# mjmyt/drone_path_planning_python

Measured on AMD Instinct MI355X. Metric: minimum-snap trajectories/sec (N drones × M segments, order 7) at 1/2/4/8 MI355X, higher is better.
Workload: dtype f64

## Files before the change

### drone_path_planning_python_amd/csrc/msnap_solve.hip

```cpp
#include "msnap_consts.h"
#include <cstdlib>

#include "msnap_internal.h"
#include "msnap_dispatch.h"
#include "msnap_sweep.h"
#include "msnap_rolled.h"

namespace msnap {


template <int K, bool GS>
__global__ void __launch_bounds__(kWave)
solve_kernel(const double *__restrict__ wp, const double *__restrict__ tt, int shared_times,
             int N, int M, double *__restrict__ coef, double *__restrict__ dur,
             int32_t *__restrict__ status, double *__restrict__ gscratch, int ntiles) {
  constexpr int NU = K - 1, NC = 2 * K;

  extern __shared__ __attribute__((aligned(16))) double lds[];

  const int lane = threadIdx.x;
  const int knots = M - 1;
  const int wpitch = (M + 1) * 4;
  const int tpitch = M + 1;

// ... 276 lines not shown
    for (int n = MCOL; n < NU; ++n) OtG[sidx(n, MCOL)] = quad_bcast<MCOL>(col[n]);
    twin_gather<NU, NS, MCOL + 1>(col, OtG);
  }
}

template <int K, int M>
__global__ void __launch_bounds__(kWave, (kTwinWaves<K, M>))
solve_kernel_twin(const double *__restrict__ wp, const double *__restrict__ tt, int shared_times,
                  int N, double *__restrict__ coef, double *__restrict__ dur,
                  int32_t *__restrict__ status, int ntiles) {
  using SW = Sweep<K>;
  using C = HermiteConsts<K>;
  constexpr int NU = SW::NU, NC = SW::NC, NS = SW::NS, KK = SW::KK, PM = SW::PM;
  static_assert(NU <= kAxes && NU >= 3, "one column of the knot blocks per axis lane (order 7: the fourth lane idles through the column work)");
  static_assert(M >= 4, "both sides own at least one knot");
  constexpr int kSlotWords = NU * kWave;
  constexpr int nL = (M - 2) / 2, nR = (M - 2) - nL;
  constexpr int H = nR;
  constexpr bool kAsym = nL != nR;
  constexpr int HA = H > 0 ? H : 1;

  extern __shared__ __attribute__((aligned(16))) double lds[];

  const int lane0 = threadIdx.x;
  constexpr int wpitch = (M + 1) * 4;
  constexpr int tpitch = M + 1;
  double *sWraw = lds;
  double *sTraw = sWraw + kTwinDrones * wpitch;
  double2 *sTr = reinterpret_cast<double2 *>(lds);
  double *sG = lds + (NC == 10 ? kTwinTrWords : 0);
  constexpr int ZL = kTwinZInLds<K, M>;
  double *sZ = sG + H * kSlotWords;
  double dsg[NU];
#pragma unroll
  for (int r = 0; r < NU; ++r) dsg[r] = (r & 1) ? 1.0 : -1.0;

  auto tile_valid = [&](int tl) {
    const int left = N - tl * kTwinDrones;
    return left < kTwinDrones ? left : kTwinDrones;
  };
  static_assert(nL >= 1, "the prefetch sits in front of segments 1 and 0 of the backward sweep, which both sides own");
  constexpr int kStoresPerSeg = (NC == 8 ? 4 : NC / 2);
  TwinStage<M> pre;
  if ((int)blockIdx.x < ntiles)
    twin_stage_load<M>(wp, tt, shared_times, blockIdx.x, tile_valid(blockIdx.x), lane0, pre);
  wait_vmcnt<0>();

  for (int tile = blockIdx.x; tile < ntiles; tile += gridDim.x) {
    int lane = lane0;
    asm volatile("" : "+v"(lane));
    const int a = lane & 3;
    const int side = (lane >> 2) & 1;
    const int blk = lane >> 2;
    const int dl = lane >> 3;
    double ca[NU];
#pragma unroll
    for (int n = 0; n < NU; ++n)
      ca[n] = a == 0 ? C::HSE[n + 1][1] : a == 1 ? C::HSE[n + 1][2] : a == 2 ? C::HSE[n + 1][3] : C::HSE[n + 1][NU];
    const int d_raw = tile * kTwinDrones + dl;
    const bool live = d_raw < N;
    const int d = live ? d_raw : N - 1;
    const int nvalid = tile_valid(tile);
    const int next = tile + gridDim.x;

    asm volatile("s_setprio 0" ::: "memory");
    wave_lds_fence();
    twin_stage_wait<M, 2 * kStoresPerSeg>(pre);
    twin_stage_store<M>(shared_times, nvalid, sWraw, sTraw, lane, pre);
    wave_lds_fence();
    store_durations(sTraw, shared_times, tpitch, M, nvalid, lane, dur + (size_t)tile * kTwinDrones * M);

    const int dloc = live ? dl : (N - 1 - tile * kTwinDrones);
    const double *lw = sWraw + dloc * wpitch + a;
    const double *lt = sTraw + (shared_times ? 0 : dloc * tpitch);
    auto Wown = [&](int i) -> double { return lw[(side ? M - i : i) * 4]; };
    auto Town = [&](int i) -> double {
      const int j = side ? M - 1 - i : i;
      return lt[j + 1] - lt[j];
    };

    double wreg[HA + 2], xreg[HA + 1], zreg[HA][NU];
    const double t0 = lt[0];
    bool nonfinite = !finite64(t0);
    bool badtime = t0 < 0.0;
#pragma unroll
    for (int i = 0; i <= H + 1; ++i) {
      wreg[i] = Wown(i);
      nonfinite |= !finite64(wreg[i]);
    }
#pragma unroll
    for (int i = 0; i <= H; ++i) {
      double T = Town(i);
      nonfinite |= !finite64(T);
      badtime |= !(T > 0.0);
      if (i == 0) {
        T = side ? T : T - t0;
        badtime |= !(T > 0.0);
      }
      xreg[i] = rcp64(T);
    }
    int in_flags = (nonfinite ? 4 : 0) | (badtime ? 2 : 0);
    asm volatile("" : "+v"(in_flags));
    wave_lds_fence();

    double xpp[PM], rz[NU], OtG[NS];
    {
      double xp[PM + 1];
      SW::powers(xreg[0], xp);
      const double dw0 = wreg[1] - wreg[0];
#pragma unroll
      for (int p = 1; p <= PM; ++p) xpp[p - 1] = xp[p];
#pragma unroll
      for (int n = 1; n <= NU; ++n) rz[n - 1] = C::HEE[n][0] * (xp[KK - n] * dw0);
#pragma unroll
      for (int e = 0; e < NS; ++e) OtG[e] = 0.0;
    }
#pragma unroll
    for (int it = 1; it <= H; ++it) {
      double xpp0[PM], rz0[NU], OtG0[NS];
      if (kAsym && it == H) {
#pragma unroll
        for (int p = 0; p < PM; ++p) xpp0[p] = xpp[p];
#pragma unroll
        for (int r = 0; r < NU; ++r) rz0[r] = rz[r];
#pragma unroll
        for (int e = 0; e < NS; ++e) OtG0[e] = OtG[e];
      }
      double xp[PM + 1];
      SW::powers(xreg[it], xp);
      const double dw = wreg[it + 1] - wreg[it];
      double S[NS], y[NU];
#pragma unroll
      for (int n = 1; n <= NU; ++n)
#pragma unroll
        for (int m = 1; m <= n; ++m)
          S[sidx(n - 1, m - 1)] =
              __builtin_fma(C::HSS[n][m], xp[KK - n - m],
                            __builtin_fma(C::HEE[n][m], xpp[KK - n - m - 1], -OtG[sidx(n - 1, m - 1)]));
#pragma unroll
      for (int n = 1; n <= NU; ++n) {
        const double tdw = xp[KK - n] * dw;
        y[n - 1] = __builtin_fma(-C::HSE[n][0], tdw, -rz[n - 1]);
        rz[n - 1] = C::HEE[n][0] * tdw;
      }
      double dinv[NU];
      in_flags |= (SW::ldl_factor(S, dinv) && (!kAsym || it <= nL || side)) ? 1 : 0;
      asm volatile("" : "+v"(in_flags));
      const double pa = a == 0 ? xp[NU] : a == 1 ? xp[NU - 1] : a == 2 ? xp[NU - 2] : xp[NU - 3];
      double g[NU];
#pragma unroll
      for (int n = 0; n < NU; ++n) g[n] = ca[n] * (n == NU - 1 ? pa : pa * xp[NU - 1 - n]);
      SW::ldl_solve(S, dinv, g);
      SW::ldl_solve(S, dinv, y);
      {
        double *gs = sG + (it - 1) * kSlotWords + lane;
#pragma unroll
        for (int r = 0; r < NU; ++r) gs[r * kWave] = g[r];
      }
      if (it <= ZL) {
#pragma unroll
        for (int r = 0; r < NU; ++r) sZ[((it - 1) * NU + r) * kWave + lane] = y[r];
      } else {
#pragma unroll
        for (int r = 0; r < NU; ++r) zreg[it - 1][r] = y[r];
      }
#pragma unroll
      for (int q = 0; q < NU - 1; ++q) {
        g[q] *= xp[NU - 1 - q];
        y[q] *= xp[NU - 1 - q];
      }
      double col[NU];
#pragma unroll
      for (int n = 0; n < NU; ++n) {
        double sg = C::HSE[1][n + 1] * g[0], sz = C::HSE[1][n + 1] * y[0];
#pragma unroll
        for (int q = 1; q < NU; ++q) {
          sg = __builtin_fma(C::HSE[q + 1][n + 1], g[q], sg);
          sz = __builtin_fma(C::HSE[q + 1][n + 1], y[q], sz);
        }
        col[n] = sg * xp[NU - n];
        rz[n] = __builtin_fma(sz, xp[NU - n], rz[n]);
      }
      twin_gather<NU, NS>(col, OtG);
#pragma unroll
      for (int p = 1; p <= PM; ++p) xpp[p - 1] = xp[p];
      if (kAsym && it == H) {
#pragma unroll
        for (int p = 0; p < PM; ++p) xpp[p] = side ? xpp[p] : xpp0[p];
#pragma unroll
        for (int r = 0; r < NU; ++r) rz[r] = side ? rz[r] : rz0[r];
#pragma unroll
        for (int e = 0; e < NS; ++e) OtG[e] = side ? OtG[e] : OtG0[e];
      }
    }

    double Sm[NS], um[NU];
#pragma unroll
    for (int r = 0; r < NU; ++r) {
      const double q = rz[r];
      um[r] = -q - dsg[r] * __shfl_xor(q, 4);
#pragma unroll
      for (int c = 0; c <= r; ++c) {
        const double p = __builtin_fma(C::HEE[r + 1][c + 1], xpp[KK - r - c - 3], -OtG[sidx(r, c)]);
        Sm[sidx(r, c)] = p + (dsg[r] * dsg[c]) * __shfl_xor(p, 4);
      }
    }
    {
      double dinv[NU];
      in_flags |= SW::ldl_factor(Sm, dinv) ? 1 : 0;
      SW::ldl_solve(Sm, dinv, um);
    }

    const int gsh = lane & ~7;
    const bool f_nonfinite = ((__ballot((in_flags & 4) != 0) >> gsh) & 0xFFull) != 0;
    const bool f_time = ((__ballot((in_flags & 2) != 0) >> gsh) & 0xFFull) != 0;
    const bool f_sing = ((__ballot((in_flags & 1) != 0) >> gsh) & 0xFFull) != 0;
    const int st = f_nonfinite ? MSNAP_ST_NONFINITE : f_time ? MSNAP_ST_TIMES : f_sing ? MSNAP_ST_SINGULAR : MSNAP_ST_OK;
    if (live && (lane & 7) == 0) status[d] = st;
    const bool bad = st != 0;

    const double qnan = __builtin_nan("");
    const double zero_or_nan = bad ? qnan : 0.0;
    TwinStorePlan plan;
    if constexpr (NC == 10) twin_store_plan(lane, plan);
    double *blkp = coef + ((size_t)d * M + (side ? M - 1 - H : H)) * (4 * NC) + (NC == 10 ? a * 2 : 0);
    const int blkstep = side ? 4 * NC : -(4 * NC);
#pragma unroll
    for (int i = 0; i < H + 2; ++i) wreg[i] = bad ? qnan : wreg[i];
    double un[NU];
#pragma unroll
    for (int r = 0; r < NU; ++r) un[r] = bad ? qnan : um[r];
#pragma unroll
    for (int it = H; it >= 0; --it) {
      if (it != 1) __builtin_amdgcn_sched_barrier(0);
      if (it == 1) {
        __builtin_amdgcn_sched_barrier(0);
        const int nx = next < ntiles ? next : ntiles - 1;
        twin_stage_load<M>(wp, tt, shared_times, nx, tile_valid(nx), lane, pre);
      }
      const bool own = !kAsym || it <= nL || side != 0;
      double u[NU];
      if (it >= 1) {
        const double2 *gsl = reinterpret_cast<const double2 *>(sG + (it - 1) * kSlotWords + blk * kAxes);
#pragma unroll
        for (int r = 0; r < NU; ++r) {
          const double2 g01 = gsl[r * (kWave / 2)], g23 = gsl[r * (kWave / 2) + 1];
          double v = (it <= ZL) ? sZ[((it >= 1 ? it - 1 : 0) * NU + r) * kWave + lane] : zreg[it >= 1 ? it - 1 : 0][r];
          v = __builtin_fma(-g01.x, un[0], v);
          v = __builtin_fma(-g01.y, un[1], v);
          v = __builtin_fma(-g23.x, un[2], v);
          if constexpr (NU == 4) v = __builtin_fma(-g23.y, un[3], v);
          u[r] = v;
        }
      } else {
#pragma unroll
        for (int r = 0; r < NU; ++r) u[r] = zero_or_nan;
      }
      double ua[NU], ub[NU];
#pragma unroll
      for (int r = 0; r < NU; ++r) {
        ua[r] = side ? dsg[r] * un[r] : u[r];
        ub[r] = side ? dsg[r] * u[r] : un[r];
      }
      const double wa = side ? wreg[it + 1] : wreg[it];
      const double wb = side ? wreg[it] : wreg[it + 1];
      double xi = xreg[it];
      asm volatile("" : "+v"(xi));
      double c[NC];
      recover_segment<K>(wa, wb - wa, xi, ua, ub, c);
      if (side == 0 && it == 0 && t0 != 0.0) taylor_shift<NC>(c, -t0);
      if (own) {
        if constexpr (NC == 10) store_twin_coalesced(sTr, blkp, lane, plan, c);
        else store_quad8_at(blkp, a, c, false);
      }
      blkp += blkstep;
#pragma unroll
      for (int r = 0; r < NU; ++r) un[r] = own ? u[r] : un[r];
    }
  }
}

constexpr int kTwistFenceHalf = 9;

__device__ __forceinline__ bool usable_duration(double T) { return __builtin_amdgcn_class(T, 0x180); }

#ifdef MSNAP_TOOLS_TIMELINE
__device__ unsigned long long g_timeline[1024 * 32];
#define MSNAP_TL(k)                                                                       \
  do {                                                                                    \
    const int row__ = (int)blockIdx.x * NW + wave;                                        \
    if (lane == 0 && row__ < 1024) {                                                      \
      g_timeline[row__ * 32 + 2 * (k)] = wall_clock64();                                  \
      g_timeline[row__ * 32 + 2 * (k) + 1] = clock64();                                   \
    }                                                                                     \
  } while (0)
#else
#define MSNAP_TL(k) do { } while (0)
#endif

template <int S, int NW>
__device__ __forceinline__ constexpr int twist_chunk_lo(int w) {
  return w * (S / NW) + (w > NW - S % NW ? w - (NW - S % NW) : 0);
}
template <int K, int MAXH, int M, int NW>
__global__ void __launch_bounds__(kWave * NW)
solve_kernel_twist(const double *__restrict__ wp, const double *__restrict__ tt, int shared_times,
                   int N, double *__restrict__ coef, double *__restrict__ dur,
                   int32_t *__restrict__ status) {
  static_assert(NW == 1 || NW == 2 || NW == 4, "one, two or four waves per tile");
  using SW = Sweep<K>;
  constexpr int NU = SW::NU, NC = SW::NC, NS = SW::NS;
  constexpr int nL = (M - 2) / 2, nR = (M - 2) - nL;
  static_assert(M >= 2 && MAXH == nR, "MAXH is the knot count of the longer side");
  constexpr int HA = MAXH > 0 ? MAXH : 1;

  extern __shared__ __attribute__((aligned(16))) double lds[];

  const int tid = threadIdx.x;
  const int lane = NW > 1 ? tid & (kWave - 1) : tid;
  const int wave = NW > 1 ? __builtin_amdgcn_readfirstlane(tid / kWave) : 0;
  const int a = lane & 3;
  const int side = (lane >> 2) & 1;
  const int dl = lane >> 3;
  constexpr int wpitch = (M + 1) * 4;
  constexpr int tpitch = M + 1;
  const int mside = side ? nR : nL;
  double *sWraw = lds;
  double *sTraw = sWraw + kTwistDrones * wpitch;
  double dsg[NU];
#pragma unroll
  for (int r = 0; r < NU; ++r) dsg[r] = (r & 1) ? 1.0 : -1.0;

  const int tile = blockIdx.x;
  {
    MSNAP_TL(0);
    const int d_raw = tile * kTwistDrones + dl;
    const bool live = d_raw < N;
    const int d = live ? d_raw : N - 1;
    const int left = N - tile * kTwistDrones;
    const int nvalid = left < kTwistDrones ? left : kTwistDrones;

    {
      constexpr int NT = kWave * NW;
      const double2 *wsrc = reinterpret_cast<const double2 *>(wp + (size_t)tile * kTwistDrones * wpitch);
      double2 *wdst = reinterpret_cast<double2 *>(sWraw);
      const int wcnt = nvalid * wpitch / 2;
      const double *tsrc = shared_times ? tt : tt + (size_t)tile * kTwistDrones * tpitch;
      const int tcnt = shared_times ? tpitch : nvalid * tpitch;
      constexpr int UW = (kTwistDrones * wpitch / 2 + NT - 1) / NT;
      constexpr int UT = (kTwistDrones * tpitch + NT - 1) / NT;
      double2 vw[UW];
      double vt[UT];
#pragma unroll
      for (int u = 0; u < UW; ++u) {
        const int e = u * NT + tid;
        vw[u] = wsrc[e < wcnt ? e : wcnt - 1];
      }
#pragma unroll
      for (int u = 0; u < UT; ++u) {
        const int f = u * NT + tid;
        vt[u] = tsrc[f < tcnt ? f : tcnt - 1];
      }
#pragma unroll
      for (int u = 0; u < UW; ++u) asm volatile("" : "+v"(vw[u].x), "+v"(vw[u].y));
#pragma unroll
      for (int u = 0; u < UT; ++u) asm volatile("" : "+v"(vt[u]));
#pragma unroll
      for (int u = 0; u < UW; ++u) {
        const int e = u * NT + tid;
        if (e < wcnt) wdst[e] = vw[u];
      }
#pragma unroll
      for (int u = 0; u < UT; ++u) {
        const int f = u * NT + tid;
        if (f < tcnt) sTraw[f] = vt[u];
      }
    }
    __syncthreads();
    MSNAP_TL(1);

    const int dloc = live ? dl : (N - 1 - tile * kTwistDrones);
    const double *lw = sWraw + dloc * wpitch + a;
    const double *lt = sTraw + (shared_times ? 0 : dloc * tpitch);
    auto Wown = [&](int i) -> double { return lw[(side ? M - i : i) * 4]; };
    auto Town = [&](int i) -> double {
      const int j = side ? M - 1 - i : i;
      return lt[j + 1] - lt[j];
    };

    constexpr bool kZReg = MAXH * NU < 3 * kTwistFenceHalf;
    double wreg[HA + 2], xreg[HA + 1], zreg[kZReg ? HA : 1][NU];
    double *sZ = sTraw + kTwistDrones * tpitch + wave * (HA * NU * kWave) + lane;
    double Greg[HA][NU][NU];
    const double t0 = lt[0];
    wreg[0] = Wown(0);
    wreg[1] = Wown(1);
    const double T0 = Town(0);
    const double T0q = side ? T0 : T0 - t0;
    constexpr bool kLean = MAXH * NU * NU <= 36;
    bool inbad = false, nonfinite = false, badtime = false;
    if constexpr (kLean) {
      inbad = !(finite64(t0) & finite64(wreg[0]) & finite64(wreg[1]) & usable_duration(T0)) | !(T0q > 0.0) | (t0 < 0.0);
    } else {
      nonfinite = !(finite64(t0) & finite64(T0) & finite64(wreg[0]) & finite64(wreg[1]));
      badtime = !(T0 > 0.0) | !(T0q > 0.0) | (t0 < 0.0);
    }
    xreg[0] = rcp64(T0q);
    SW sw;
    sw.init(xreg[0], wreg[1] - wreg[0]);

    double xpc[SW::PM + 1], dwc = 0.0;
    auto ahead = [&](int it, double (&xp)[SW::PM + 1], double &dw) {
      wreg[it + 1] = Wown(it + 1);
      const double Tit = Town(it);
      if constexpr (kLean) {
        inbad |= !(usable_duration(Tit) & finite64(wreg[it + 1]));
      } else {
        nonfinite |= !finite64(Tit) | !finite64(wreg[it + 1]);
        badtime |= !(Tit > 0.0);
      }
      xreg[it] = rcp64(Tit);
      SW::powers(xreg[it], xp);
      dw = wreg[it + 1] - wreg[it];
    };
    if (MAXH >= 1) ahead(1, xpc, dwc);
    bool singular = false;
    auto knot_step = [&](int it) {
      double G[NU][NU], z[NU];
      typename SW::Knot k;
      SW::knot_geom_xp(xpc, dwc, sw.E, sw.re, k);
      const bool ok = sw.chain(k, G, z);
      singular |= !ok & (it <= mside);
#pragma unroll
      for (int e = 0; e < NS; ++e) sw.E[e] = k.E[e];
#pragma unroll
      for (int r = 0; r < NU; ++r) {
        sw.re[r] = k.re[r];
        if constexpr (kZReg) zreg[it - 1][r] = z[r];
        else sZ[((it - 1) * NU + r) * kWave] = z[r];
#pragma unroll
        for (int c = 0; c < NU; ++c) Greg[it - 1][r][c] = G[r][c];
      }
    };
#pragma unroll
    for (int it = 1; it <= MAXH; ++it) {
      if (it < MAXH) {
        double xpn[SW::PM + 1], dwn;
        ahead(it + 1, xpn, dwn);
        knot_step(it);
        dwc = dwn;
#pragma unroll
        for (int q = 0; q <= SW::PM; ++q) xpc[q] = xpn[q];
        if constexpr (MAXH * NU >= 3 * kTwistFenceHalf) __builtin_amdgcn_sched_barrier(0);
      } else if (nL == nR) {
        knot_step(it);
      } else {
        double E0[NS], G0[NS], r0[NU], z0[NU];
#pragma unroll
        for (int e = 0; e < NS; ++e) { E0[e] = sw.E[e]; G0[e] = sw.OtG[e]; }
#pragma unroll
        for (int r = 0; r < NU; ++r) { r0[r] = sw.re[r]; z0[r] = sw.Otz[r]; }
        knot_step(it);
#pragma unroll
        for (int e = 0; e < NS; ++e) { sw.E[e] = side ? sw.E[e] : E0[e]; sw.OtG[e] = side ? sw.OtG[e] : G0[e]; }
#pragma unroll
        for (int r = 0; r < NU; ++r) { sw.re[r] = side ? sw.re[r] : r0[r]; sw.Otz[r] = side ? sw.Otz[r] : z0[r]; }
      }
    }

    MSNAP_TL(2);
    double Sm[NS], um[NU];
#pragma unroll
    for (int r = 0; r < NU; ++r) {
      const double q = sw.re[r] + sw.Otz[r];
      um[r] = -q - dsg[r] * row_xor4_f64(q);
#pragma unroll
      for (int c = 0; c <= r; ++c) {
        const double p = sw.E[sidx(r, c)] - sw.OtG[sidx(r, c)];
        Sm[sidx(r, c)] = p + (dsg[r] * dsg[c]) * row_xor4_f64(p);
      }
    }
    {
      double dinv[NU];
      singular |= SW::ldl_factor(Sm, dinv);
      SW::ldl_solve(Sm, dinv, um);
    }

    auto classify = [&]() -> int {
      const int gsh = lane & ~7;
      const bool f_nonfinite = ((__ballot(nonfinite) >> gsh) & 0xFFull) != 0;
      const bool f_time = ((__ballot(badtime) >> gsh) & 0xFFull) != 0;
      const bool f_sing = ((__ballot(singular) >> gsh) & 0xFFull) != 0;
      return f_nonfinite ? MSNAP_ST_NONFINITE : f_time ? MSNAP_ST_TIMES : f_sing ? MSNAP_ST_SINGULAR : MSNAP_ST_OK;
    };
    auto put_status = [&](int st) {
      if (live && (lane & 7) == 0 && wave == NW - 1) status[d] = st;
    };
    double zero_or_nan = 0.0;
    double un[NU];
    auto poison = [&](bool bad) {
      const double qnan = __builtin_nan("");
      zero_or_nan = bad ? qnan : 0.0;
#pragma unroll
      for (int i = 0; i < MAXH + 2; ++i) wreg[i] = bad ? qnan : wreg[i];
#pragma unroll
      for (int r = 0; r < NU; ++r) un[r] = bad ? qnan : um[r];
    };
    if constexpr (kLean) {
      int st = MSNAP_ST_OK;
#pragma unroll
      for (int r = 0; r < NU; ++r) un[r] = um[r];
      if (__builtin_expect(__builtin_amdgcn_ballot_w64(inbad | singular) != 0, 0)) {
        asm volatile("" ::: "memory");
        const double T0r = Town(0);
        nonfinite = !(finite64(t0) & finite64(T0r) & finite64(wreg[0]) & finite64(wreg[1]));
        badtime = !(T0r > 0.0) | !((side ? T0r : T0r - t0) > 0.0) | (t0 < 0.0);
#pragma unroll
        for (int it = 1; it <= MAXH; ++it) {
          const double Tit = Town(it);
          nonfinite |= !finite64(Tit) | !finite64(wreg[it + 1]);
          badtime |= !(Tit > 0.0);
        }
        st = classify();
        poison(st != 0);
      }
      put_status(st);
    } else {
      const int st = classify();
      put_status(st);
      poison(st != 0);
    }

    MSNAP_TL(3);
    const int lo = twist_chunk_lo<MAXH + 1, NW>(wave), hi = twist_chunk_lo<MAXH + 1, NW>(wave + 1) - 1;
#pragma unroll
    for (int it = MAXH; it >= 0; --it) {
      if (NW > 1 && (it < lo || hi < lo)) break;
      if (it <= nL || side) {
        double u[NU];
        if (it >= 1) {
#pragma unroll
          for (int r = 0; r < NU; ++r) {
            double v;
            if constexpr (kZReg) v = zreg[it >= 1 ? it - 1 : 0][r];
            else v = sZ[((it >= 1 ? it - 1 : 0) * NU + r) * kWave];
#pragma unroll
            for (int c = 0; c < NU; ++c) v = __builtin_fma(-Greg[it >= 1 ? it - 1 : 0][r][c], un[c], v);
            u[r] = v;
          }
        } else {
#pragma unroll
          for (int r = 0; r < NU; ++r) u[r] = zero_or_nan;
        }
        if (NW == 1 || it <= hi) {
        double ua[NU], ub[NU];
#pragma unroll
        for (int r = 0; r < NU; ++r) {
          ua[r] = side ? dsg[r] * un[r] : u[r];
          ub[r] = side ? dsg[r] * u[r] : un[r];
        }
        const double wa = side ? wreg[it + 1] : wreg[it];
        const double wb = side ? wreg[it] : wreg[it + 1];
        double c[NC];
        recover_segment<K>(wa, wb - wa, xreg[it], ua, ub, c);
        if (side == 0 && it == 0 && t0 != 0.0) taylor_shift<NC>(c, -t0);
        const int seg = side ? M - 1 - it : it;
        {
          double *o = coef + (((size_t)d * M + seg) * 4 + a) * NC;
#pragma unroll
          for (int m = 0; m < NC; m += 2) *reinterpret_cast<double2 *>(o + m) = make_double2(c[m], c[m + 1]);
        }
        }
#pragma unroll
        for (int r = 0; r < NU; ++r) un[r] = u[r];
      }
      if constexpr (MAXH * NU >= 3 * kTwistFenceHalf) __builtin_amdgcn_sched_barrier(0);
    }
    __builtin_amdgcn_sched_barrier(0);
    store_durations<kTwistDrones * M, kWave * NW>(sTraw, shared_times, tpitch, M, nvalid, tid,
                                                  dur + (size_t)tile * kTwistDrones * M);
    MSNAP_TL(4);
  }
}

static SolveKnobs solve_knobs(const msnap_ctx *ctx) {
  return {ctx->n_cu, ctx->no_twist, ctx->no_twin, ctx->twist_max_drones, ctx->twin_max_drones, ctx->twist_waves,
          ctx->solve_grid_waves};
}

template <int K>
static int launch_solve_k(msnap_ctx *ctx, int N, int M, const double *wp, const double *t, int shared,
                          double *coef, double *dur, int32_t *status) {
  const SolvePlan p = plan_solve(solve_knobs(ctx), K, N, M);
  if (p.slab_bytes > 0) {
    int rc = ensure(ctx, ctx->scratch, p.slab_bytes);
    if (rc) return rc;
  }
  solve_plan_name(p, ctx->last_kernel, sizeof(ctx->last_kernel));
  const dim3 grid(p.grid), block(p.block);
  bool found = true;
  switch (p.family) {
    case SolveFamily::twist:
      found = dispatch_range<2, twist_max_seg(K)>(M, [&](auto seg) {
        constexpr int MM = decltype(seg)::value;
        auto launch = [&](auto waves) {
          hipLaunchKernelGGL((solve_kernel_twist<K, twist_half(MM), MM, decltype(waves)::value>), grid, block,
                             p.lds_bytes, ctx->stream, wp, t, shared, N, coef, dur, status);
        };
        if (p.waves == 4) launch(std::integral_constant<int, 4>{});
        else if (p.waves == 2) launch(std::integral_constant<int, 2>{});
        else launch(std::integral_constant<int, 1>{});
      });
      break;
    case SolveFamily::twin:
      found = dispatch_range<kTwinMinSeg, twin_max_seg(K)>(M, [&](auto seg) {
        hipLaunchKernelGGL((solve_kernel_twin<K, decltype(seg)::value>), grid, block, p.lds_bytes, ctx->stream, wp, t,
                           shared, N, coef, dur, status, p.tiles);
      });
      break;
    case SolveFamily::reg:
      if (p.seg == kRegMaxSeg)
        hipLaunchKernelGGL((solve_kernel_reg<K, kRegMaxSeg>), grid, block, p.lds_bytes, ctx->stream, wp, t, shared, N, M,
                           coef, dur, status, p.tiles);
      else
        hipLaunchKernelGGL((solve_kernel_reg<K, kRegMaxSeg2>), grid, block, p.lds_bytes, ctx->stream, wp, t, shared, N, M,
                           coef, dur, status, p.tiles);
      break;
    case SolveFamily::rolled:
      if (p.slab_bytes > 0)
        hipLaunchKernelGGL((solve_kernel<K, true>), grid, block, p.lds_bytes, ctx->stream, wp, t, shared, N, M, coef, dur,
                           status, (double *)ctx->scratch.p, p.tiles);
      else
        hipLaunchKernelGGL((solve_kernel<K, false>), grid, block, p.lds_bytes, ctx->stream, wp, t, shared, N, M, coef,
                           dur, status, (double *)nullptr, p.tiles);
      break;
  }
  if (!found) return MSNAP_EINVAL;
  MSNAP_HIP(ctx, hipGetLastError());
  return MSNAP_OK;
}

bool solve_uses_global_scratch(const msnap_ctx *ctx, int n_seg) {
  return plan_solve(solve_knobs(ctx), ctx->khalf, 1, n_seg).slab_bytes > 0;
}

#ifdef MSNAP_TOOLS_TIMELINE
extern "C" int msnap_debug_read_timeline(unsigned long long *out, int n_words) {
  if (hipDeviceSynchronize() != hipSuccess) return MSNAP_EHIP;
  return hipMemcpyFromSymbol(out, HIP_SYMBOL(g_timeline), (size_t)n_words * 8) == hipSuccess ? MSNAP_OK : MSNAP_EHIP;
}
#endif

int solve_kernel_setup(msnap_ctx *ctx) {
  MSNAP_HIP(ctx, hipFuncSetAttribute(reinterpret_cast<const void *>(&solve_kernel<4, false>),
                                     hipFuncAttributeMaxDynamicSharedMemorySize, (int)kMaxLdsBytes));
  MSNAP_HIP(ctx, hipFuncSetAttribute(reinterpret_cast<const void *>(&solve_kernel<5, false>),
                                     hipFuncAttributeMaxDynamicSharedMemorySize, (int)kMaxLdsBytes));
  return MSNAP_OK;
}

int launch_solve(msnap_ctx *ctx, int n_drones, int n_seg, const double *wp, const double *t,
                 int shared_times, double *coef, double *dur, int32_t *status) {
  if (n_drones == 0) return MSNAP_OK;
  if (ctx->khalf == 4)
    return launch_solve_k<4>(ctx, n_drones, n_seg, wp, t, shared_times, coef, dur, status);
  return launch_solve_k<5>(ctx, n_drones, n_seg, wp, t, shared_times, coef, dur, status);
}

}
```

### drone_path_planning_python_amd/csrc/msnap_sweep.h

```cpp
#pragma once

#include "msnap_consts.h"
#include "msnap_internal.h"
#include "msnap_solve_plan.h"
#include "msnap_energy.h"
#include "msnap_wave.h"

namespace msnap {

__device__ __forceinline__ constexpr int sidx(int r, int c) {
  return r * (r + 1) / 2 + c;
}

__device__ __forceinline__ double rcp64(double v) {
  double r = __builtin_amdgcn_rcp(v);
  double e = __builtin_fma(-v, r, 1.0);
  r = __builtin_fma(r, e, r);
  e = __builtin_fma(-v, r, 1.0);
  r = __builtin_fma(r, e, r);
  return r;
}

__device__ __forceinline__ bool finite64(double v) { return __builtin_isfinite(v); }

template <int K>
struct Sweep {
  static constexpr int NU = K - 1;
  static constexpr int NC = 2 * K;
  static constexpr int KK = 2 * K - 1;
  static constexpr int NS = NU * (NU + 1) / 2;
  static constexpr int PM = 2 * K - 2;
  using C = HermiteConsts<K>;

  double E[NS], re[NU];
  double OtG[NS], Otz[NU];
  bool singular;

  __device__ __forceinline__ static void powers(double x, double (&xp)[PM + 1]) {
    xp[0] = 1.0;
    xp[1] = x;
#pragma unroll
    for (int p = 2; p <= PM; ++p) xp[p] = xp[p - 1] * x;
  }

  __device__ __forceinline__ void end_side(const double (&xp)[PM + 1], double dw) {
#pragma unroll
    for (int n = 1; n <= NU; ++n) {
#pragma unroll
      for (int m = 1; m <= n; ++m) E[sidx(n - 1, m - 1)] = C::HEE[n][m] * xp[KK - n - m];
      re[n - 1] = (C::HEE[n][0] * xp[KK - n]) * dw;
    }
  }

  __device__ __forceinline__ void init(double x, double dw) {
    double xp[PM + 1];
    powers(x, xp);
    end_side(xp, dw);
    singular = false;
#pragma unroll
    for (int r = 0; r < NU; ++r) Otz[r] = 0.0;
#pragma unroll
    for (int e = 0; e < NS; ++e) OtG[e] = 0.0;
  }

  struct Knot {
    double D[NS], O[NU][NU], yb[NU], E[NS], re[NU];
  };

  __device__ __forceinline__ static void knot_geom(double x, double dw, const double (&Eprev)[NS],
                                                   const double (&reprev)[NU], Knot &k) {
    double xp[PM + 1];
    powers(x, xp);
    knot_geom_xp(xp, dw, Eprev, reprev, k);
  }

  __device__ __forceinline__ static void knot_geom_xp(const double (&xp)[PM + 1], double dw,
                                                      const double (&Eprev)[NS], const double (&reprev)[NU],
                                                      Knot &k) {
#pragma unroll
    for (int n = 1; n <= NU; ++n) {
#pragma unroll
      for (int m = 1; m <= n; ++m) {
        k.D[sidx(n - 1, m - 1)] = __builtin_fma(C::HSS[n][m], xp[KK - n - m], Eprev[sidx(n - 1, m - 1)]);
        k.E[sidx(n - 1, m - 1)] = C::HEE[n][m] * xp[KK - n - m];
      }
      k.yb[n - 1] = __builtin_fma(C::HSE[n][0] * xp[KK - n], dw, reprev[n - 1]);
      k.re[n - 1] = (C::HEE[n][0] * xp[KK - n]) * dw;
#pragma unroll
      for (int m = 1; m <= NU; ++m) k.O[n - 1][m - 1] = C::HSE[n][m] * xp[KK - n - m];
    }
  }

  __device__ __forceinline__ static bool ldl_factor(double (&S)[NS], double (&dinv)[NU]) {
    bool bad = false;
#pragma unroll
    for (int j = 0; j < NU; ++j) {
      double dj = S[sidx(j, j)];
#pragma unroll
      for (int p = 0; p < j; ++p) dj = __builtin_fma(-S[sidx(j, p)] * dinv[p], S[sidx(j, p)], dj);
      bad |= !(dj > 0.0) | !finite64(dj);
      dinv[j] = rcp64(dj);
#pragma unroll
      for (int r = j + 1; r < NU; ++r) {
        double v = S[sidx(r, j)];
#pragma unroll
        for (int p = 0; p < j; ++p) v = __builtin_fma(-S[sidx(r, p)] * dinv[p], S[sidx(j, p)], v);
        S[sidx(r, j)] = v;
      }
    }
#pragma unroll
    for (int r = 1; r < NU; ++r)
#pragma unroll
      for (int p = 0; p < r; ++p) S[sidx(r, p)] *= dinv[p];
    return bad;
  }

  __device__ __forceinline__ static void ldl_solve(const double (&S)[NS], const double (&dinv)[NU], double (&v)[NU]) {
#pragma unroll
    for (int r = 1; r < NU; ++r)
#pragma unroll
      for (int p = 0; p < r; ++p) v[r] = __builtin_fma(-S[sidx(r, p)], v[p], v[r]);
#pragma unroll
    for (int r = 0; r < NU; ++r) v[r] *= dinv[r];
#pragma unroll
    for (int r = NU - 2; r >= 0; --r)
#pragma unroll
      for (int p = r + 1; p < NU; ++p) v[r] = __builtin_fma(-S[sidx(p, r)], v[p], v[r]);
  }

  __device__ __forceinline__ bool chain(const Knot &k, double (&G)[NU][NU], double (&z)[NU]) {
    double S[NS], y[NU];
#pragma unroll
    for (int n = 0; n < NU; ++n) {
#pragma unroll
      for (int m = 0; m <= n; ++m) S[sidx(n, m)] = k.D[sidx(n, m)] - OtG[sidx(n, m)];
      y[n] = -k.yb[n] - Otz[n];
    }

    double dinv[NU];
    const bool bad = ldl_factor(S, dinv);

#pragma unroll
    for (int c = 0; c <= NU; ++c) {
      double v[NU];
#pragma unroll
      for (int r = 0; r < NU; ++r) v[r] = (c < NU) ? k.O[r][c < NU ? c : 0] : y[r];
      ldl_solve(S, dinv, v);
#pragma unroll
      for (int r = 0; r < NU; ++r) {
        if (c < NU) G[r][c < NU ? c : 0] = v[r];
        else z[r] = v[r];
      }
    }

#pragma unroll
    for (int n = 0; n < NU; ++n) {
#pragma unroll
      for (int m = 0; m <= n; ++m) {
        double v = 0.0;
#pragma unroll
        for (int q = 0; q < NU; ++q) v = __builtin_fma(k.O[q][n], G[q][m], v);
        OtG[sidx(n, m)] = v;
      }
      double w = 0.0;
#pragma unroll
      for (int q = 0; q < NU; ++q) w = __builtin_fma(k.O[q][n], z[q], w);
      Otz[n] = w;
    }
    return !bad;
  }

  __device__ __forceinline__ void step(double x, double dw, double (&G)[NU][NU], double (&z)[NU]) {
    Knot k;
    knot_geom(x, dw, E, re, k);
    singular |= !chain(k, G, z);
#pragma unroll
    for (int e = 0; e < NS; ++e) E[e] = k.E[e];
#pragma unroll
    for (int r = 0; r < NU; ++r) re[r] = k.re[r];
  }
};

template <int K>
__device__ __forceinline__ void recover_segment(double wi, double dwi, double xi, const double (&u)[K - 1],
                                                const double (&un)[K - 1], double (&c)[2 * K]) {
  using C = HermiteConsts<K>;
  double xq[K + 1];
  xq[0] = 1.0;
#pragma unroll
  for (int m = 1; m <= K; ++m) xq[m] = xq[m - 1] * xi;
  c[0] = wi;
#pragma unroll
  for (int n = 1; n < K; ++n) c[n] = u[n - 1] * C::INVFACT[n];
  double es[K], ee[K];
#pragma unroll
  for (int n = 1; n < K; ++n) {
    es[n] = (n == K - 1) ? u[n - 1] : xq[K - 1 - n] * u[n - 1];
    ee[n] = (n == K - 1) ? un[n - 1] : xq[K - 1 - n] * un[n - 1];
  }
  const double dwx = dwi * xq[K - 1];
#pragma unroll
  for (int m = 0; m < K; ++m) {
    double acc = C::CE[m][0] * dwx;
#pragma unroll
    for (int n = 1; n < K; ++n) {
      acc = __builtin_fma(C::CS[m][n], es[n], acc);
      acc = __builtin_fma(C::CE[m][n], ee[n], acc);
    }
    c[K + m] = acc * xq[m + 1];
  }
}

template <int NC>
__device__ __forceinline__ void taylor_shift(double (&c)[NC], double h) {
#pragma unroll
  for (int j = 0; j < NC - 1; ++j)
#pragma unroll
    for (int q = NC - 2; q >= j; --q) c[q] = __builtin_fma(h, c[q + 1], c[q]);
}

#define MSNAP_SEG_BASE(coef, tile, M, i, NC) ((coef) + ((size_t)(tile) * kDronesPerWave * (M) + (i)) * (4 * (NC)))
#define MSNAP_SEG_STRIDE(M, NC) ((size_t)(M) * 4 * (NC))
template <int NC>
__device__ __forceinline__ void store_segment_coalesced(double2 *sTr, double *__restrict__ seg_base,
                                                        size_t drone_stride, int nvalid, int lane,
                                                        double (&c)[NC], bool bad) {
  constexpr int NJ = NC / 2;
  if (__builtin_expect(__builtin_amdgcn_ballot_w64(bad) != 0, 0)) {
    asm volatile("" ::: "memory");
#pragma unroll
    for (int m = 0; m < NC; ++m) c[m] = bad ? __builtin_nan("") : c[m];
  }
#pragma unroll
  for (int j = 0; j < NJ; ++j) sTr[j * kTrPitch + lane] = make_double2(c[2 * j], c[2 * j + 1]);
  __builtin_amdgcn_fence(__ATOMIC_RELEASE, "wavefront", "local");
  __builtin_amdgcn_wave_barrier();
  __builtin_amdgcn_fence(__ATOMIC_ACQUIRE, "wavefront", "local");
#pragma unroll
  for (int q = 0; q < NJ; ++q) {
    const int s = q * kWave + lane;
    const int drone = s / (4 * NJ);
    const int within = s - drone * (4 * NJ);
    const int a2 = within / NJ;
    const int j2 = within - a2 * NJ;
    const double2 v = sTr[j2 * kTrPitch + drone * 4 + a2];
    const int dst = drone < nvalid ? drone : nvalid - 1;
    *reinterpret_cast<double2 *>(seg_base + (size_t)dst * drone_stride + within * 2) = v;
  }
  __builtin_amdgcn_fence(__ATOMIC_RELEASE, "wavefront", "local");
  __builtin_amdgcn_wave_barrier();
}

#define MSNAP_QCND(d, s0, s1, QP) \
  "v_cndmask_b32_dpp %" #d ", %" #s0 ", %" #s1 ", vcc quad_perm:" QP " row_mask:0xf bank_mask:0xf\n\t"
#define MSNAP_QSTAGE(QP, out, src, keep, mask)                                                                     \
  asm("s_nop 1\n\ts_mov_b64 vcc, %16\n\t" MSNAP_QCND(0, 8, 17, QP) MSNAP_QCND(1, 9, 18, QP) MSNAP_QCND(2, 10, 19, QP) \
          MSNAP_QCND(3, 11, 20, QP) MSNAP_QCND(4, 12, 21, QP) MSNAP_QCND(5, 13, 22, QP) MSNAP_QCND(6, 14, 23, QP)      \
              MSNAP_QCND(7, 15, 24, QP)                                                                            \
      : "=&v"(out[0]), "=&v"(out[1]), "=&v"(out[2]), "=&v"(out[3]), "=&v"(out[4]), "=&v"(out[5]), "=&v"(out[6]),    \
        "=&v"(out[7])                                                                                              \
      : "v"(src[0]), "v"(src[1]), "v"(src[2]), "v"(src[3]), "v"(src[4]), "v"(src[5]), "v"(src[6]), "v"(src[7]),     \
        "s"(mask), "v"(keep[0]), "v"(keep[1]), "v"(keep[2]), "v"(keep[3]), "v"(keep[4]), "v"(keep[5]), "v"(keep[6]), \
        "v"(keep[7])                                                                                               \
      : "vcc")
template <int STAGE>
__device__ __forceinline__ void quad_stage(uint32_t (&a)[8], uint32_t (&b)[8], unsigned long long bit) {
  uint32_t na[8], nb[8];
  const unsigned long long nbit = ~bit;
  if constexpr (STAGE == 1) {
    MSNAP_QSTAGE("[1,0,3,2]", nb, a, b, bit);
    MSNAP_QSTAGE("[1,0,3,2]", na, b, a, nbit);
  } else {
    MSNAP_QSTAGE("[2,3,0,1]", nb, a, b, bit);
    MSNAP_QSTAGE("[2,3,0,1]", na, b, a, nbit);
  }
#pragma unroll
  for (int k = 0; k < 8; ++k) {
    a[k] = na[k];
    b[k] = nb[k];
  }
}
#undef MSNAP_QSTAGE
#undef MSNAP_QCND

__device__ __forceinline__ void store_quad8_at(double *__restrict__ blk, int a, const double (&c)[8], bool bad) {
  double p[8];
#pragma unroll
  for (int k = 0; k < 8; ++k) p[k] = c[k];
  if (__builtin_expect(__builtin_amdgcn_ballot_w64(bad) != 0, 0)) {
    asm volatile("" ::: "memory");
#pragma unroll
    for (int k = 0; k < 8; ++k) p[k] = bad ? __builtin_nan("") : p[k];
  }
  auto lo = [](double v) { return (uint32_t)__double2loint(v); };
  auto hi = [](double v) { return (uint32_t)__double2hiint(v); };
  uint32_t A[8] = {lo(p[0]), hi(p[0]), lo(p[1]), hi(p[1]), lo(p[4]), hi(p[4]), lo(p[5]), hi(p[5])};
  uint32_t B[8] = {lo(p[2]), hi(p[2]), lo(p[3]), hi(p[3]), lo(p[6]), hi(p[6]), lo(p[7]), hi(p[7])};
  quad_stage<1>(A, B, __builtin_amdgcn_ballot_w64((a & 1) != 0));
  uint32_t A2[8] = {A[0], A[1], A[2], A[3], B[0], B[1], B[2], B[3]};
  uint32_t B2[8] = {A[4], A[5], A[6], A[7], B[4], B[5], B[6], B[7]};
  quad_stage<2>(A2, B2, __builtin_amdgcn_ballot_w64((a & 2) != 0));
  uint4 *o = reinterpret_cast<uint4 *>(blk + a * 2);
  o[0] = make_uint4(A2[0], A2[1], A2[2], A2[3]);
  o[4] = make_uint4(A2[4], A2[5], A2[6], A2[7]);
  o[8] = make_uint4(B2[0], B2[1], B2[2], B2[3]);
  o[12] = make_uint4(B2[4], B2[5], B2[6], B2[7]);
}

__device__ __forceinline__ void store_segment_quad8(double *__restrict__ seg_base, size_t drone_stride,
                                                    int nvalid, int lane, const double (&c)[8], bool bad) {
  const int dl = lane >> 2;
  store_quad8_at(seg_base + (size_t)(dl < nvalid ? dl : nvalid - 1) * drone_stride, lane & 3, c, bad);
}

template <int MAXCNT = 0, int STRIDE = kWave>
__device__ __forceinline__ void store_durations(const double *sTraw, int shared_times, int tpitch, int M,
                                                int nvalid, int lane, double *__restrict__ dur_tile) {
  const int cnt = nvalid * M;
  auto one = [&](int e) {
    if (e < cnt) {
      const int dl = e / M;
      const int i = e - dl * M;
      const double *lt = sTraw + (shared_times ? 0 : dl * tpitch);
      dur_tile[e] = lt[i + 1] - lt[i];
    }
  };
  if constexpr (MAXCNT > 0) {
#pragma unroll
    for (int e0 = 0; e0 < MAXCNT; e0 += STRIDE) one(e0 + lane);
  } else {
    for (int e0 = 0; e0 < cnt; e0 += STRIDE) one(e0 + lane);
  }
}

__device__ __forceinline__ int drone_status(bool nonfinite, bool badtime, bool singular) {
  int flags = (nonfinite ? 4 : 0) | (badtime ? 2 : 0) | (singular ? 1 : 0);
  flags |= __shfl_xor(flags, 1);
  flags |= __shfl_xor(flags, 2);
  return (flags & 4) ? MSNAP_ST_NONFINITE : (flags & 2) ? MSNAP_ST_TIMES : (flags & 1) ? MSNAP_ST_SINGULAR : MSNAP_ST_OK;
}

__device__ __forceinline__ void stage_inputs(const double *__restrict__ wp, const double *__restrict__ tt,
                                             int shared_times, int tile, int nvalid, int wpitch, int tpitch,
                                             double *sWraw, double *sTraw, int lane) {
  const double2 *wsrc = reinterpret_cast<const double2 *>(wp + (size_t)tile * kDronesPerWave * wpitch);
  double2 *wdst = reinterpret_cast<double2 *>(sWraw);
  const int wcnt = nvalid * wpitch / 2;
  const double *tsrc = shared_times ? tt : tt + (size_t)tile * kDronesPerWave * tpitch;
  const int tcnt = shared_times ? tpitch : nvalid * tpitch;
  constexpr int UW = 8, UT = 4;
  for (int e0 = 0, f0 = 0; e0 < wcnt || f0 < tcnt; e0 += UW * kWave, f0 += UT * kWave) {
    double2 vw[UW];
    double vt[UT];
#pragma unroll
    for (int u = 0; u < UW; ++u) {
      const int e = e0 + u * kWave + lane;
      vw[u] = wsrc[e < wcnt ? e : wcnt - 1];
    }
#pragma unroll
    for (int u = 0; u < UT; ++u) {
      const int f = f0 + u * kWave + lane;
      vt[u] = tsrc[f < tcnt ? f : tcnt - 1];
    }
#pragma unroll
    for (int u = 0; u < UW; ++u) asm volatile("" : "+v"(vw[u].x), "+v"(vw[u].y));
#pragma unroll
    for (int u = 0; u < UT; ++u) asm volatile("" : "+v"(vt[u]));
#pragma unroll
    for (int u = 0; u < UW; ++u) {
      const int e = e0 + u * kWave + lane;
      if (e < wcnt) wdst[e] = vw[u];
    }
#pragma unroll
    for (int u = 0; u < UT; ++u) {
      const int f = f0 + u * kWave + lane;
      if (f < tcnt) sTraw[f] = vt[u];
    }
  }
}

typedef unsigned int u32x4 __attribute__((ext_vector_type(4)));
template <int MAXM>
struct StageRegsAsm {
  static constexpr int UW = (MAXM + 2) / 2;
  static constexpr int UT = (MAXM + 4) / 4;
  u32x4 vw[UW];
  double vt[UT];
};

template <int MAXM>
__device__ __forceinline__ void stage_load_asm(const double *__restrict__ wp, const double *__restrict__ tt,
                                               int shared_times, int tile, int nvalid, int wpitch, int tpitch,
                                               int lane, StageRegsAsm<MAXM> &r) {
  const double2 *wsrc = reinterpret_cast<const double2 *>(wp + (size_t)tile * kDronesPerWave * wpitch);
  const int wcnt = nvalid * wpitch / 2;
  const double *tsrc = shared_times ? tt : tt + (size_t)tile * kDronesPerWave * tpitch;
  const int tcnt = shared_times ? tpitch : nvalid * tpitch;
#pragma unroll
  for (int u = 0; u < StageRegsAsm<MAXM>::UW; ++u) {
    const int e = u * kWave + lane;
    const double2 *p = wsrc + (e < wcnt ? e : wcnt - 1);
    asm volatile("global_load_dwordx4 %0, %1, off" : "=v"(r.vw[u]) : "v"(p) : "memory");
  }
#pragma unroll
  for (int u = 0; u < StageRegsAsm<MAXM>::UT; ++u) {
    const int f = u * kWave + lane;
    const double *p = tsrc + (f < tcnt ? f : tcnt - 1);
    asm volatile("global_load_dwordx2 %0, %1, off" : "=v"(r.vt[u]) : "v"(p) : "memory");
  }
}

template <int MAXM, int YOUNGER>
__device__ __forceinline__ void stage_wait_asm(StageRegsAsm<MAXM> &r) {
  wait_vmcnt<YOUNGER>();
#pragma unroll
  for (int u = 0; u < StageRegsAsm<MAXM>::UW; ++u) asm volatile("" : "+v"(r.vw[u]));
#pragma unroll
  for (int u = 0; u < StageRegsAsm<MAXM>::UT; ++u) asm volatile("" : "+v"(r.vt[u]));
}

template <int MAXM>
__device__ __forceinline__ void stage_store_asm(int shared_times, int nvalid, int wpitch, int tpitch,
                                                double *sWraw, double *sTraw, int lane, StageRegsAsm<MAXM> &r) {
  u32x4 *wdst = reinterpret_cast<u32x4 *>(sWraw);
  const int wcnt = nvalid * wpitch / 2;
  const int tcnt = shared_times ? tpitch : nvalid * tpitch;
#pragma unroll
  for (int u = 0; u < StageRegsAsm<MAXM>::UW; ++u) {
    const int e = u * kWave + lane;
    if (e < wcnt) wdst[e] = r.vw[u];
  }
#pragma unroll
  for (int u = 0; u < StageRegsAsm<MAXM>::UT; ++u) {
    const int f = u * kWave + lane;
    if (f < tcnt) sTraw[f] = r.vt[u];
  }
}

__device__ __forceinline__ void wave_lds_fence() {
  __builtin_amdgcn_fence(__ATOMIC_RELEASE, "wavefront", "local");
  __builtin_amdgcn_wave_barrier();
  __builtin_amdgcn_fence(__ATOMIC_ACQUIRE, "wavefront", "local");
}

template <int SRC>
__device__ __forceinline__ double quad_bcast(double v) {
  int lo = __double2loint(v), hi = __double2hiint(v);
  lo = __builtin_amdgcn_mov_dpp(lo, SRC * 0x55, 0xf, 0xf, true);
  hi = __builtin_amdgcn_mov_dpp(hi, SRC * 0x55, 0xf, 0xf, true);
  return __hiloint2double(hi, lo);
}

}
```

Measured before the change: 63.75 million.

## Load Hermite constants into SGPRs from a constant table via scalar loads

Moves the non-inline Hermite f64 constants used by the sweep and segment recovery into a deduplicated __constant__ table. The kernel loads them into scalar registers with s_load_dwordx* early, overlapping those loads with the LDS staging, and prefetches the recovery constants before the backward pass. Literal f64 constants otherwise have to be materialised in VGPRs or as 64-bit literal operands, so this aims to cut instruction count and vector register pressure. The cost is SGPR pressure, inline-asm waitcnt handling, and extra scalar-memory latency, and it only applies to the small configurations selected by kTab.

```diff
diff --git a/drone_path_planning_python_amd/csrc/msnap_solve.hip b/drone_path_planning_python_amd/csrc/msnap_solve.hip
--- a/drone_path_planning_python_amd/csrc/msnap_solve.hip
+++ b/drone_path_planning_python_amd/csrc/msnap_solve.hip
@@ -602,6 +602,54 @@
 __device__ __forceinline__ constexpr int twist_chunk_lo(int w) {
   return w * (S / NW) + (w > NW - S % NW ? w - (NW - S % NW) : 0);
 }
+__constant__ TwistConstImage g_twist_consts = twist_const_image();
+
+typedef double f64x2 __attribute__((ext_vector_type(2)));
+typedef double f64x4 __attribute__((ext_vector_type(4)));
+typedef double f64x8 __attribute__((ext_vector_type(8)));
+template <int OFF, int N>
+__device__ __forceinline__ void sload_f64(const double *src, double (&dst)[N]) {
+  if constexpr (N - OFF >= 8) {
+    f64x8 v;
+    asm volatile("s_load_dwordx16 %0, %1, %2" : "=s"(v) : "s"(src), "i"(OFF * 8));
+#pragma unroll
+    for (int q = 0; q < 8; ++q) dst[OFF + q] = v[q];
+    sload_f64<OFF + 8>(src, dst);
+  } else if constexpr (N - OFF >= 4) {
+    f64x4 v;
+    asm volatile("s_load_dwordx8 %0, %1, %2" : "=s"(v) : "s"(src), "i"(OFF * 8));
+#pragma unroll
+    for (int q = 0; q < 4; ++q) dst[OFF + q] = v[q];
+    sload_f64<OFF + 4>(src, dst);
+  } else if constexpr (N - OFF >= 2) {
+    f64x2 v;
+    asm volatile("s_load_dwordx4 %0, %1, %2" : "=s"(v) : "s"(src), "i"(OFF * 8));
+    dst[OFF] = v[0];
+    dst[OFF + 1] = v[1];
+    sload_f64<OFF + 2>(src, dst);
+  } else if constexpr (N - OFF == 1) {
+    asm volatile("s_load_dwordx2 %0, %1, %2" : "=s"(dst[OFF]) : "s"(src), "i"(OFF * 8));
+  }
+}
+template <int OFF, int NL>
+__device__ __forceinline__ void sload_touch(const double *src, unsigned (&t)[NL]) {
+  if constexpr (OFF < NL) {
+    asm volatile("s_load_dword %0, %1, %2" : "=s"(t[OFF]) : "s"(src), "i"(OFF * 64));
+    sload_touch<OFF + 1>(src, t);
+  }
+}
+template <int NL>
+__device__ __forceinline__ void touch_wait(unsigned (&t)[NL]) {
+#pragma unroll
+  for (int s = 0; s < NL; ++s) asm volatile("" : "+s"(t[s]));
+}
+template <int N>
+__device__ __forceinline__ void sload_wait(double (&v)[N]) {
+  asm volatile("s_waitcnt lgkmcnt(0)" ::: "memory");
+#pragma unroll
+  for (int s = 0; s < N; ++s) asm volatile("" : "+s"(v[s]));
+}
+
 template <int K, int MAXH, int M, int NW>
 __global__ void __launch_bounds__(kWave * NW)
 solve_kernel_twist(const double *__restrict__ wp, const double *__restrict__ tt, int shared_times,
@@ -632,6 +680,16 @@
   for (int r = 0; r < NU; ++r) dsg[r] = (r & 1) ? 1.0 : -1.0;
 
   const int tile = blockIdx.x;
+  constexpr bool kTab = MAXH * (K - 1) * (K - 1) <= 36 && !(K == 5 && M == 4);
+  constexpr bool kTabRec = kTab && K == 4;
+  using HC = std::conditional_t<kTab, TableHermite<K, kTabRec>, LiteralHermite<K>>;
+  HC hc;
+  constexpr int kRecLines = kTabRec ? (TwistConstLayout<K>::n_rec * 8 + 63) / 64 : 1;
+  unsigned rec_touch[kRecLines];
+  if constexpr (kTab) {
+    sload_f64<0>(g_twist_consts.v + TwistConstLayout<K>::sweep_at, hc.sw);
+    if constexpr (kTabRec) sload_touch<0>(g_twist_consts.v + TwistConstLayout<K>::rec_at, rec_touch);
+  }
   {
     MSNAP_TL(0);
     const int d_raw = tile * kTwistDrones + dl;
@@ -678,6 +736,10 @@
     }
     __syncthreads();
     MSNAP_TL(1);
+    if constexpr (kTab) {
+      sload_wait(hc.sw);
+      if constexpr (kTabRec) touch_wait(rec_touch);
+    }
 
     const int dloc = live ? dl : (N - 1 - tile * kTwistDrones);
     const double *lw = sWraw + dloc * wpitch + a;
@@ -707,7 +769,7 @@
     }
     xreg[0] = rcp64(T0q);
     SW sw;
-    sw.init(xreg[0], wreg[1] - wreg[0]);
+    sw.init(xreg[0], wreg[1] - wreg[0], hc);
 
     double xpc[SW::PM + 1], dwc = 0.0;
     auto ahead = [&](int it, double (&xp)[SW::PM + 1], double &dw) {
@@ -728,7 +790,7 @@
     auto knot_step = [&](int it) {
       double G[NU][NU], z[NU];
       typename SW::Knot k;
-      SW::knot_geom_xp(xpc, dwc, sw.E, sw.re, k);
+      SW::knot_geom_xp(xpc, dwc, sw.E, sw.re, k, hc);
       const bool ok = sw.chain(k, G, z);
       singular |= !ok & (it <= mside);
 #pragma unroll
@@ -769,6 +831,7 @@
     }
 
     MSNAP_TL(2);
+    if constexpr (kTabRec) sload_f64<0>(g_twist_consts.v + TwistConstLayout<K>::rec_at, hc.rc);
     double Sm[NS], um[NU];
 #pragma unroll
     for (int r = 0; r < NU; ++r) {
@@ -832,6 +895,7 @@
     }
 
     MSNAP_TL(3);
+    if constexpr (kTabRec) sload_wait(hc.rc);
     const int lo = twist_chunk_lo<MAXH + 1, NW>(wave), hi = twist_chunk_lo<MAXH + 1, NW>(wave + 1) - 1;
 #pragma unroll
     for (int it = MAXH; it >= 0; --it) {
@@ -862,7 +926,12 @@
         const double wa = side ? wreg[it + 1] : wreg[it];
         const double wb = side ? wreg[it] : wreg[it + 1];
         double c[NC];
-        recover_segment<K>(wa, wb - wa, xreg[it], ua, ub, c);
+        if constexpr (kTabRec) {
+          if (it <= nL) recover_segment<K>(wa, wb - wa, xreg[it], ua, ub, c, hc);
+          else recover_segment<K>(wa, wb - wa, xreg[it], ua, ub, c);
+        } else {
+          recover_segment<K>(wa, wb - wa, xreg[it], ua, ub, c);
+        }
         if (side == 0 && it == 0 && t0 != 0.0) taylor_shift<NC>(c, -t0);
         const int seg = side ? M - 1 - it : it;
         {
diff --git a/drone_path_planning_python_amd/csrc/msnap_sweep.h b/drone_path_planning_python_amd/csrc/msnap_sweep.h
--- a/drone_path_planning_python_amd/csrc/msnap_sweep.h
+++ b/drone_path_planning_python_amd/csrc/msnap_sweep.h
@@ -1,6 +1,7 @@
 #pragma once
 
 #include "msnap_consts.h"
+#include "msnap_twist_consts.h"
 #include "msnap_internal.h"
 #include "msnap_solve_plan.h"
 #include "msnap_energy.h"
@@ -22,6 +23,34 @@
 }
 
 __device__ __forceinline__ bool finite64(double v) { return __builtin_isfinite(v); }
+
+template <int K>
+struct LiteralHermite {
+  using C = HermiteConsts<K>;
+  __device__ __forceinline__ double hss(int n, int m) const { return C::HSS[n][m]; }
+  __device__ __forceinline__ double hee(int n, int m) const { return C::HEE[n][m]; }
+  __device__ __forceinline__ double hse(int n, int m) const { return C::HSE[n][m]; }
+  __device__ __forceinline__ double cs(int m, int n) const { return C::CS[m][n]; }
+  __device__ __forceinline__ double ce(int m, int n) const { return C::CE[m][n]; }
+  __device__ __forceinline__ double invfact(int n) const { return C::INVFACT[n]; }
+};
+
+template <int K, bool REC = true>
+struct TableHermite {
+  using C = HermiteConsts<K>;
+  using L = TwistConstLayout<K>;
+  static constexpr int NSW = L::n_sweep, NRC = REC ? L::n_rec : 0;
+  double sw[NSW], rc[REC ? L::n_rec : 1];
+  __device__ __forceinline__ static double pick(int code, double lit, const double *tab) {
+    return code == 0 ? lit : tab[code - 1];
+  }
+  __device__ __forceinline__ double hss(int n, int m) const { return pick(TwistMapOf<K>::map.hss[n][m], C::HSS[n][m], sw); }
+  __device__ __forceinline__ double hee(int n, int m) const { return pick(TwistMapOf<K>::map.hee[n][m], C::HEE[n][m], sw); }
+  __device__ __forceinline__ double hse(int n, int m) const { return pick(TwistMapOf<K>::map.hse[n][m], C::HSE[n][m], sw); }
+  __device__ __forceinline__ double cs(int m, int n) const { return pick(!REC ? 0 : TwistMapOf<K>::map.cs[m][n], C::CS[m][n], rc); }
+  __device__ __forceinline__ double ce(int m, int n) const { return pick(!REC ? 0 : TwistMapOf<K>::map.ce[m][n], C::CE[m][n], rc); }
+  __device__ __forceinline__ double invfact(int n) const { return pick(!REC ? 0 : TwistMapOf<K>::map.inv[n], C::INVFACT[n], rc); }
+};
 
 template <int K>
 struct Sweep {
@@ -43,19 +72,21 @@
     for (int p = 2; p <= PM; ++p) xp[p] = xp[p - 1] * x;
   }
 
-  __device__ __forceinline__ void end_side(const double (&xp)[PM + 1], double dw) {
+  template <class P = LiteralHermite<K>>
+  __device__ __forceinline__ void end_side(const double (&xp)[PM + 1], double dw, P hc = P()) {
 #pragma unroll
     for (int n = 1; n <= NU; ++n) {
 #pragma unroll
-      for (int m = 1; m <= n; ++m) E[sidx(n - 1, m - 1)] = C::HEE[n][m] * xp[KK - n - m];
-      re[n - 1] = (C::HEE[n][0] * xp[KK - n]) * dw;
-    }
-  }
-
-  __device__ __forceinline__ void init(double x, double dw) {
+      for (int m = 1; m <= n; ++m) E[sidx(n - 1, m - 1)] = hc.hee(n, m) * xp[KK - n - m];
+      re[n - 1] = (hc.hee(n, 0) * xp[KK - n]) * dw;
+    }
+  }
+
+  template <class P = LiteralHermite<K>>
+  __device__ __forceinline__ void init(double x, double dw, P hc = P()) {
     double xp[PM + 1];
     powers(x, xp);
-    end_side(xp, dw);
+    end_side(xp, dw, hc);
     singular = false;
 #pragma unroll
     for (int r = 0; r < NU; ++r) Otz[r] = 0.0;
@@ -74,20 +105,21 @@
     knot_geom_xp(xp, dw, Eprev, reprev, k);
   }
 
+  template <class P = LiteralHermite<K>>
   __device__ __forceinline__ static void knot_geom_xp(const double (&xp)[PM + 1], double dw,
                                                       const double (&Eprev)[NS], const double (&reprev)[NU],
-                                                      Knot &k) {
+                                                      Knot &k, P hc = P()) {
 #pragma unroll
     for (int n = 1; n <= NU; ++n) {
 #pragma unroll
       for (int m = 1; m <= n; ++m) {
-        k.D[sidx(n - 1, m - 1)] = __builtin_fma(C::HSS[n][m], xp[KK - n - m], Eprev[sidx(n - 1, m - 1)]);
-        k.E[sidx(n - 1, m - 1)] = C::HEE[n][m] * xp[KK - n - m];
+        k.D[sidx(n - 1, m - 1)] = __builtin_fma(hc.hss(n, m), xp[KK - n - m], Eprev[sidx(n - 1, m - 1)]);
+        k.E[sidx(n - 1, m - 1)] = hc.hee(n, m) * xp[KK - n - m];
       }
-      k.yb[n - 1] = __builtin_fma(C::HSE[n][0] * xp[KK - n], dw, reprev[n - 1]);
-      k.re[n - 1] = (C::HEE[n][0] * xp[KK - n]) * dw;
-#pragma unroll
-      for (int m = 1; m <= NU; ++m) k.O[n - 1][m - 1] = C::HSE[n][m] * xp[KK - n - m];
+      k.yb[n - 1] = __builtin_fma(hc.hse(n, 0) * xp[KK - n], dw, reprev[n - 1]);
+      k.re[n - 1] = (hc.hee(n, 0) * xp[KK - n]) * dw;
+#pragma unroll
+      for (int m = 1; m <= NU; ++m) k.O[n - 1][m - 1] = hc.hse(n, m) * xp[KK - n - m];
     }
   }
 
@@ -181,17 +213,16 @@
   }
 };
 
-template <int K>
+template <int K, class P = LiteralHermite<K>>
 __device__ __forceinline__ void recover_segment(double wi, double dwi, double xi, const double (&u)[K - 1],
-                                                const double (&un)[K - 1], double (&c)[2 * K]) {
-  using C = HermiteConsts<K>;
+                                                const double (&un)[K - 1], double (&c)[2 * K], P hc = P()) {
   double xq[K + 1];
   xq[0] = 1.0;
 #pragma unroll
   for (int m = 1; m <= K; ++m) xq[m] = xq[m - 1] * xi;
   c[0] = wi;
 #pragma unroll
-  for (int n = 1; n < K; ++n) c[n] = u[n - 1] * C::INVFACT[n];
+  for (int n = 1; n < K; ++n) c[n] = u[n - 1] * hc.invfact(n);
   double es[K], ee[K];
 #pragma unroll
   for (int n = 1; n < K; ++n) {
@@ -201,11 +232,11 @@
   const double dwx = dwi * xq[K - 1];
 #pragma unroll
   for (int m = 0; m < K; ++m) {
-    double acc = C::CE[m][0] * dwx;
+    double acc = hc.ce(m, 0) * dwx;
 #pragma unroll
     for (int n = 1; n < K; ++n) {
-      acc = __builtin_fma(C::CS[m][n], es[n], acc);
-      acc = __builtin_fma(C::CE[m][n], ee[n], acc);
+      acc = __builtin_fma(hc.cs(m, n), es[n], acc);
+      acc = __builtin_fma(hc.ce(m, n), ee[n], acc);
     }
     c[K + m] = acc * xq[m + 1];
   }
diff --git a/drone_path_planning_python_amd/csrc/msnap_twist_consts.h b/drone_path_planning_python_amd/csrc/msnap_twist_consts.h
--- /dev/null
+++ b/drone_path_planning_python_amd/csrc/msnap_twist_consts.h
@@ -0,0 +1,85 @@
+#pragma once
+
+#include "msnap_consts.h"
+
+namespace msnap {
+
+template <int K>
+struct TwistConstMap {
+  static constexpr int NU = K - 1;
+  static constexpr int kMaxSweep = 5 * K * K, kMaxRec = 2 * K * K + K;
+  int hss[K][K] = {}, hee[K][K] = {}, hse[K][K] = {};
+  int cs[K][K] = {}, ce[K][K] = {}, inv[K] = {};
+  double sweep[kMaxSweep] = {}, rec[kMaxRec] = {};
+  int n_sweep = 0, n_rec = 0;
+
+  static constexpr bool inline_operand(double v) {
+    const double m = v < 0 ? -v : v;
+    return m == 0.5 || m == 1.0 || m == 2.0 || m == 4.0;
+  }
+  static constexpr int place(double v, double *tab, int &n) {
+    if (inline_operand(v)) return 0;
+    int s = 0;
+    while (s < n && tab[s] != v) ++s;
+    if (s == n) tab[n++] = v;
+    return s + 1;
+  }
+  constexpr TwistConstMap() {
+    using C = HermiteConsts<K>;
+    for (int n = 1; n <= NU; ++n) {
+      for (int m = 1; m <= n; ++m) {
+        hss[n][m] = place(C::HSS[n][m], sweep, n_sweep);
+        hee[n][m] = place(C::HEE[n][m], sweep, n_sweep);
+      }
+      hse[n][0] = place(C::HSE[n][0], sweep, n_sweep);
+      hee[n][0] = place(C::HEE[n][0], sweep, n_sweep);
+      for (int m = 1; m <= NU; ++m) hse[n][m] = place(C::HSE[n][m], sweep, n_sweep);
+    }
+    for (int n = 1; n < K; ++n) inv[n] = place(C::INVFACT[n], rec, n_rec);
+    for (int m = 0; m < K; ++m) {
+      ce[m][0] = place(C::CE[m][0], rec, n_rec);
+      for (int n = 1; n < K; ++n) {
+        cs[m][n] = place(C::CS[m][n], rec, n_rec);
+        ce[m][n] = place(C::CE[m][n], rec, n_rec);
+      }
+    }
+  }
+};
+
+template <int K>
+struct TwistMapOf {
+  static constexpr TwistConstMap<K> map{};
+};
+
+constexpr int twist_pad8(int n) { return (n + 7) / 8 * 8; }
+template <int K>
+constexpr int twist_set_words() {
+  return twist_pad8(TwistMapOf<K>::map.n_sweep) + twist_pad8(TwistMapOf<K>::map.n_rec);
+}
+template <int K>
+struct TwistConstLayout {
+  static_assert(K == 4 || K == 5, "the twisted solve has order 7 and order 9 instances");
+  static constexpr int n_sweep = TwistMapOf<K>::map.n_sweep, n_rec = TwistMapOf<K>::map.n_rec;
+  static constexpr int sweep_at = (K == 4) ? 0 : twist_set_words<4>();
+  static constexpr int rec_at = sweep_at + twist_pad8(n_sweep);
+  static constexpr int end = rec_at + twist_pad8(n_rec);
+};
+constexpr int kTwistConstWords = TwistConstLayout<5>::end;
+
+struct alignas(64) TwistConstImage {
+  double v[kTwistConstWords];
+};
+template <int K>
+constexpr void twist_image_fill(TwistConstImage &t) {
+  using L = TwistConstLayout<K>;
+  for (int s = 0; s < L::n_sweep; ++s) t.v[L::sweep_at + s] = TwistMapOf<K>::map.sweep[s];
+  for (int s = 0; s < L::n_rec; ++s) t.v[L::rec_at + s] = TwistMapOf<K>::map.rec[s];
+}
+constexpr TwistConstImage twist_const_image() {
+  TwistConstImage t{};
+  twist_image_fill<4>(t);
+  twist_image_fill<5>(t);
+  return t;
+}
+
+}
```

Measured after the change: 65.31 million (median of 6 runs). 2.5% higher.
